# batra-mlp-lab/visdial

Hardware: AMD Instinct MI355X
Metric: QA-rounds/sec training mn-att-ques-im-hist+disc (batch 20x10x100) (higher is better)
Workload: dtype f32 operands and results; the option recurrence multiplies the EXACT 3-way bf16 split of both operands (9 bf16 MFMA products per fp32 product, f32 accumulate: fp32-grade, errors at the f32 MFMA's own level) -- its two step kernels and its weight-gradient contraction; f32 MFMA (v_mfma_f32_32x32x2_f32

## Files before the change

### visdial_amd/csrc/gemm_ops.hip

```cpp
#include "gemm_core.h"
#include "split_core.h"

using CfgBigDB = GemmCfg<4, 1, 4, 32>;
using CfgBig = GemmCfg<4, 1, 4, 16, 0, 3>;
using CfgSmall = GemmCfg<1, 4, 1, 32, 0, 3>;

static inline bool use_small(int M, int N) {
  return (long)vd_cdiv(M, CfgBig::BM) * vd_cdiv(N, CfgBig::BN) < 48;
}

static int check_align(const void* p, long ld, const char* what) {
  if (((uintptr_t)p & 15) != 0 || (ld & 3) != 0) {
    vd_set_error("%s: pointer must be 16-byte aligned and leading dimension a multiple of 4 (ld=%ld)", what, ld);
    return VD_ERR_ARG;
  }
  return VD_OK;
}

__global__ void colsum_kernel(const float* __restrict__ X, long ld, int M, int N, int rows_per_block,
                              float* __restrict__ out) {
  const int col = blockIdx.x * blockDim.x + threadIdx.x;
  if (col >= N) return;
  const int r0 = blockIdx.y * rows_per_block;
  const int r1 = min(M, r0 + rows_per_block);
// ... 349 lines not shown
  const int* tok_mask;
  static constexpr bool HAS_DEAD = true;
  __device__ __forceinline__ bool dead(int row_base, int ) const { return tok_mask[row_base] == 0; }
};
static_assert(CfgSmall::BM == VD_LSTM_FWD_TILE_SMALL && CfgBig::BM == VD_LSTM_FWD_TILE_BIG, "the projection's row tiles are the step kernels'");

int vd_gemm_nn_live_p(const float* A, int64_t lda, const float* B, int64_t ldb, const float* bias, float* C, int64_t ldc, int M, int N, int K,
                      const int32_t* tok_mask, int row_tile, hipStream_t s) {
  VD_CHECK_ARG(A && B && C && tok_mask && M >= 0 && N >= 0 && K >= 0 && (K % 4 == 0 || lda >= (K + 3) / 4 * 4) && N % 4 == 0 &&
                   (row_tile == CfgSmall::BM || row_tile == CfgBig::BM),
               "vd_gemm_nn (live rows): bad args M=%d N=%d K=%d row tile %d", M, N, K, row_tile);
  if (int rc = check_align(A, lda, "vd_gemm_nn (live rows) A")) return rc;
  if (int rc = check_align(B, ldb, "vd_gemm_nn (live rows) B")) return rc;
  SrcRow a{A, lda};
  SrcK b{B, ldb};
  if (row_tile == CfgSmall::BM) {
    EpiStoreLive<1> e{{C, ldc, bias, VD_ACT_NONE, 0}, tok_mask};
    return launch_gemm<CfgSmall>(M, N, K, 1, a, b, e, s);
  }
  EpiStoreLive<4> e{{C, ldc, bias, VD_ACT_NONE, 0}, tok_mask};
  return launch_gemm<CfgBig>(M, N, K, 1, a, b, e, s);
}

extern "C" {

int vd_gemm_tn_acc(const float* A, int64_t lda, const float* B, int64_t ldb, float* C, int64_t ldc, int M,
                   int N, int K, int flags, void* stream) {
  VD_CHECK_ARG(A && B && C && M >= 0 && N >= 0 && K >= 0 && (M % 4 == 0 || lda >= (M + 3) / 4 * 4) &&
                   (N % 4 == 0 || ldb >= (N + 3) / 4 * 4),
               "vd_gemm_tn_acc: bad args M=%d N=%d K=%d", M, N, K);
  if (int rc = check_align(A, lda, "vd_gemm_tn_acc A")) return rc;
  if (int rc = check_align(B, ldb, "vd_gemm_tn_acc B")) return rc;
  if (K == 0) return VD_OK;
  SrcK a{A, lda}, b{B, ldb};
  EpiAtomic<4> e{C, ldc};
  const long tiles = (long)vd_cdiv(M, CfgBig::BM) * vd_cdiv(N, CfgBig::BN);
  if ((flags & VD_FLAG_SPLIT9) && !(flags & VD_FLAG_BF16) && vd_tn_split_tiles(M, N) && K >= 8192 &&
      16L * lda * 4 < (1L << 31) && 16L * ldb * 4 < (1L << 31)) {
    const int K1 = K & ~15;
    if (int rc = launch_gemm_split_tn<9>(M, N, K1, A, lda, B, ldb, C, ldc, (hipStream_t)stream)) return rc;
    if (K1 == K) return VD_OK;
    SrcK a2{A + (long)K1 * lda, lda}, b2{B + (long)K1 * ldb, ldb};
    return launch_gemm<GemmCfg<4, 1, 4, 16, 0, 4, 41984>>(M, N, K - K1, 1, a2, b2, e, (hipStream_t)stream);
  }
  const bool kmaj = !(flags & VD_FLAG_BF16) && vd_tn_kmajor_fits(M, N, K);
  if (kmaj && K % 16 != 0) {
// ... 126 lines not shown
```

### visdial_amd/csrc/paths.h

```cpp
#pragma once
#include "common.h"

static inline int vd_precision_flags(int lstmBf16) {
  switch (lstmBf16) {
    case 0: return 0;
    case 1: return VD_FLAG_BF16;
    case 3: return VD_FLAG_SPLIT3;
    case 6: return VD_FLAG_SPLIT6;
    case 9: return VD_FLAG_SPLIT9;
    default: return -1;
  }
}
static inline int vd_split_nprod(int flags) {
  return (flags & VD_FLAG_SPLIT9) ? 9 : (flags & VD_FLAG_SPLIT6) ? 6 : (flags & VD_FLAG_SPLIT3) ? 3 : 0;
}

constexpr long VD_THROUGHPUT_ROWS = 2048;
constexpr int VD_LSTM_FWD_TILE_BIG = 128, VD_LSTM_FWD_TILE_SMALL = 32;
static inline int vd_lstm_fwd_row_tile(long N) { return N >= VD_THROUGHPUT_ROWS ? VD_LSTM_FWD_TILE_BIG : VD_LSTM_FWD_TILE_SMALL; }
static inline bool vd_lstm_glds_fwd_fits(long N, int H) { return N >= VD_THROUGHPUT_ROWS && H % 32 == 0 && N * H * 4 < (1L << 32); }
static inline bool vd_lstm_glds_bwd_fits(long N, int H) { return N >= VD_THROUGHPUT_ROWS && H % 32 == 0 && N * 4 * H * 4 < (1L << 32); }
static inline bool vd_lstm_bf16_fits(long N, int H) { return N >= VD_THROUGHPUT_ROWS && H % 32 == 0; }
static inline bool vd_lstm_c16_fits(long N, int H) { return N >= VD_THROUGHPUT_ROWS && H % 128 == 0; }

static inline bool vd_tn_kmajor_fits(long M, long N, long K) { return M % 128 == 0 && N % 128 == 0 && K >= 1024; }
constexpr int VD_SPLIT_TN_BM = 256, VD_SPLIT_TN_BN = 128;
static inline bool vd_tn_split_tiles(long M, long N) { return M % VD_SPLIT_TN_BM == 0 && N % VD_SPLIT_TN_BN == 0; }

static inline bool vd_wgrad_group_fits(bool sorted_rows, long M, long N, int flags) {
  return sorted_rows && M % 128 == 0 && N % 128 == 0 && !(flags & VD_FLAG_BF16);
}

static inline bool vd_img_split_ok(long rows, int H, int Kc) {
  return rows >= 128 && H % 16 == 0 && Kc % 16 == 0 && rows * (H > Kc ? H : Kc) * 4 < (1L << 32);
}

static inline bool vd_lhood_fused_fits(long rows, long ldh, long V, long ldw, int H) {
  return H >= 64 && H % 16 == 0 && V >= 128 && ldh % 4 == 0 && ldw % 4 == 0 && rows * ldh * 4 < (1L << 32) && V * ldw * 4 < (1L << 32);
}
static inline bool vd_lhood_prefix_fits(int T, long rows) { return T >= 1 && T < 256 && rows >= 1; }
```

### visdial_amd/csrc/rt_core.h

```cpp
#pragma once
#include <math.h>
#include <stdarg.h>
#include <stdlib.h>
#include <string.h>

#include <algorithm>
#include <map>
#include <memory>
#include <numeric>
#include <random>
#include <string>
#include <vector>

#include "../../include/visdial_hip.h"
#include "common.h"
#include "paths.h"
#include "rt_switches.h"
#include "wgrad_plan.h"

static_assert(VD_OK == 0 && VD_ERR_ARG == -1, "rt_switches.h returns the two as literals: it includes no common.h");

int vd_lstm2_forward_p(const vd_lstm2_fwd_t* st, int nstacks, int H, int flags, hipStream_t stream);
int vd_lstm2_backward_p(const vd_lstm2_bwd_t* st, int nstacks, int H, int flags, hipStream_t stream);

// ... 1 lines not shown
int vd_img_common_forward_p(const float* pre, const uint8_t* mask1, const float* xdrop, const float* Wc, const float* bc, const float* qc,
                            const uint8_t* mask2, float* iqc, int N, int R, int S2, int H, int Kc, float scale, int flags, hipStream_t stream);
int vd_img_tr_backward_p(const float* dz, const float* Wc, const float* p, const float* datt, const uint8_t* mask1, float* dpre, int N, int R,
                         int S2, int H, int Kc, float scale, int flags, hipStream_t stream);
int vd_img_common_wgrad_p(const float* dz, const float* pre, const uint8_t* mask1, const float* xdrop, float* dWc, int N, int R, int S2, int H,
                          int Kc, float scale, int flags, hipStream_t stream);

int vd_img_att_forward_p(const float* iqc, const float* wa, const float* ba, const float* pre, const uint8_t* mask1, const float* u0, float* p,
                         float* u1, int N, int R, int S2, int H, int Kc, float scale, const int32_t* cnt, hipStream_t stream);
int vd_img_att_backward_p(float* iqc_dz, const float* wa, const float* pre, const uint8_t* mask1, const uint8_t* mask2, const float* p,
                          const float* datt, float* dwa, float* dba, float* dqc, float* work, int N, int R, int S2, int H, int Kc, float scale,
                          const int32_t* cnt, hipStream_t stream);

int vd_mn_attention_round_p(const float* Q, int64_t q_ld, const float* Hm, float* P, float* hAtt, float* Qout, int B, int R, int r, int H,
                            hipStream_t stream);
int vd_hrea_attention_round_p(const float* sq, const float* sh, const float* Hm, float* P, float* att, int B, int R, int r, int H,
                              hipStream_t stream);
int vd_round_embed_p(const float* emb, const int32_t* tok, int T, int N, int R, int r, int32_t* tok_r, float* x, int E, hipStream_t stream);
int vd_rows_cat_p(float* dst, int64_t dst_ld, const float* const* src, const int64_t* ld, const int* cols, int nparts, int64_t rows,
                  hipStream_t stream);

int vd_gemm_nn_live_p(const float* A, int64_t lda, const float* B, int64_t ldb, const float* bias, float* C, int64_t ldc, int M, int N, int K,
                      const int32_t* tok_mask, int row_tile, hipStream_t stream);
int vd_lhood_order_p(const int32_t* tok_in, const int32_t* target, int T, int64_t rows, int C, int32_t* perm, int32_t* rep, int32_t* tok_in_s,
                     int32_t* target_s, int32_t* work, int32_t* info, hipStream_t stream);
int64_t vd_lhood_order_work_ints(int T, int64_t rows);
int vd_lhood_sum_p(const float* nll, const int32_t* act, int64_t n_act, int T, int64_t rows, int C, const int32_t* perm, float* out, int64_t ldo,
                   hipStream_t stream);

int vd_lhood_lse_p(const float* h, int64_t ldh, int64_t rows, const int32_t* act, int64_t n_act, const float* W, int64_t ldw, const float* bias,
                   int V, int H, float* lse, hipStream_t stream);
int vd_lhood_edge_sum_p(const float* h, int64_t ldh, const int32_t* node_row, const float* lse, const int32_t* enode, const int32_t* etgt, int T,
                        int64_t rows, int C, const float* W, int64_t ldw, const float* bias, int H, float* out, int64_t ldo, hipStream_t stream);

int vd_sample_draw_trunc_p(const float* logits, int64_t ld, int64_t rows, int V, int32_t* tok, const double* uniforms, double temperature,
                           int top_k, double top_p, int step, int beam_len, int end_token, int32_t* hist, double* loglik, int32_t* status,
                           hipStream_t stream);

int vd_beam_advance_p(const int32_t* top_idx, const float* top_val, int rounds, int k, int G, float lambda, int step, int beam_len,
                      int end_token, double* scores, const int32_t* hist_in, int32_t* hist_out, int32_t* src, int32_t* next_tok,
                      double* best_score, int32_t* best_len, int32_t* best_hist, const double* lp, hipStream_t stream);
int vd_beam_topk_ban_p(const float* logits, int64_t ld, int64_t rows, int V, const int32_t* tok, int k, const int32_t* hist, int beam_len,
                       int step, int min_len, int no_repeat, int end_token, int32_t* top_idx, float* top_val, hipStream_t stream);

int vd_beam_rollout_append_p(const int32_t* answers, int beam_len, int end_token, const int32_t* ques, int Tq, int dialogs, int R, int r,
                             int32_t* hist_tok, int32_t* hist_sorted, const int32_t* inv, int Th, hipStream_t stream, int concat_end = 0);
// ... 230 lines not shown
  return VD_OK;
}

template <class T>
int ws_get(vd_model* m, const std::string& key, size_t count, T** out) {
  void* p = nullptr;
  VD_TRY(dev_get(m->ws, key, count * sizeof(T), &p));
  *out = static_cast<T*>(p);
  return VD_OK;
}

inline void add_lstm(vd_model* m, const std::string& name, long D, long H) {
  m->spec.push_back(Tensor{name + ".W", 0, D + H, 4 * H, 1});
  m->spec.push_back(Tensor{name + ".b", 0, 1, 4 * H, 2});
}
inline void add_linear(vd_model* m, const std::string& name, long in, long out) {
  m->spec.push_back(Tensor{name + ".W", 0, out, in, 3});
  m->spec.push_back(Tensor{name + ".b", 0, 1, out, 4});
}
inline std::string hop_sfx(int i) { return i == 0 ? std::string() : std::to_string(i + 1); }

inline float* Wp(vd_model* m, const std::string& n) { return m->W + m->spec[m->index.at(n)].off; }
inline float* Gp(vd_model* m, const std::string& n) { return m->G + m->spec[m->index.at(n)].off; }

inline int fork_stream(vd_model* m, hipStream_t from, hipStream_t side) {
  if (side == from) return VD_OK;
  hipEvent_t e = m->ev_pool[m->ev_next++ % m->ev_pool.size()];
  VD_HIP(hipEventRecord(e, from));
  VD_HIP(hipStreamWaitEvent(side, e, 0));
  return VD_OK;
}
inline int join_stream(vd_model* m, hipStream_t side, hipStream_t to) { return fork_stream(m, side, to); }
inline hipStream_t side_stream(vd_model* m, hipStream_t cur) { return m->streams ? m->s_side : cur; }
inline int wg_fork(vd_model* m, hipStream_t cur, hipStream_t* out) {
  *out = cur;
  if (!m->wg_active || !m->s_wg) return VD_OK;
  VD_TRY(fork_stream(m, cur, m->s_wg));
  m->wg_used = true;
  *out = m->s_wg;
  return VD_OK;
}

constexpr int VD_WGRAD_CHUNKS = 768, VD_WGRAD_MIN_KSTEPS = 32;
inline void wgrad_begin(vd_model* m) {
  m->wgrad.clear();
  m->wgrad_open = true;
// ... 284 lines not shown
    if (T > 1 && grouped(h, H, gates + (long)N * 4 * H, dWh, 1)) {
    } else if (by_rows && !(T > 1 && dense_fits(H, (long)(T - 1) * N))) {
      if (rows->n_act1 > 0)
        VD_TRY(vd_gemm_tn_rows_acc(h, H, rows->prev1, gates, 4 * H, rows->act1, dWh, 4 * H, (int)H, (int)(4 * H), rows->n_act1, s));
    } else if (T > 1) {
      VD_TRY(vd_gemm_tn_acc(h, H, gates + (long)N * 4 * H, 4 * H, dWh, 4 * H, (int)H, (int)(4 * H), (T - 1) * N, wg_flags(H), s));
    }
    if (h0) VD_TRY(vd_gemm_tn_acc(h0, H, gates, 4 * H, dWh, 4 * H, (int)H, (int)(4 * H), N, 0, s));
    VD_TRY(vd_colsum_acc(gates, 4 * H, (int)TN, (int)(4 * H), Gp(m, name + ".b"), s));
    if (dxs) dxs->assign(parts.size(), nullptr);
    long roff = 0;
    for (size_t i = 0; i < parts.size(); ++i) {
      if (grouped(xs[i], parts[i], gates, dW + roff * 4 * H, 0)) {
      } else if (by_rows && !dense_fits(parts[i], TN)) {
        if (rows->n_act > 0)
          VD_TRY(vd_gemm_tn_rows_acc(xs[i], parts[i], rows->act, gates, 4 * H, rows->act, dW + roff * 4 * H, 4 * H, (int)parts[i],
                                     (int)(4 * H), rows->n_act, s));
      } else {
        VD_TRY(vd_gemm_tn_acc(xs[i], parts[i], gates, 4 * H, dW + roff * 4 * H, 4 * H, (int)parts[i], (int)(4 * H), (int)TN, wg_flags(parts[i]), s));
      }
      if (need_dx.empty() || need_dx[i]) {
        float* dx;
        VD_TRY(ws_get(m, name + ".dx" + std::to_string(i), (size_t)TN * parts[i], &dx));
        VD_TRY(vd_gemm_nt(gates, 4 * H, Wx(m) + roff * 4 * H, 4 * H, nullptr, dx, parts[i], (int)TN, (int)parts[i], (int)(4 * H),
                          VD_ACT_NONE, 0, s));
        if (dxs) (*dxs)[i] = dx;
      }
      roff += parts[i];
    }
    return VD_OK;
  }
  int backward(vd_model* m, hipStream_t s, const float* dh_seq, const float* dh_last, const std::vector<bool>& need_dx,
               std::vector<float*>* dxs) {
    if (gradPrevOutput) {
      if (!dh_last) dh_last = gradPrevOutput;
      else {
        float* t;
        VD_TRY(ws_get(m, name + ".dhl", (size_t)N * H, &t));
        VD_TRY(vd_axpby(dh_last, gradPrevOutput, t, (long)N * H, 1.f, 1.f, s));
        dh_last = t;
      }
    }
    const float* dc_last = userNextGradCell;
    gradPrevOutput = userNextGradCell = nullptr;
    float *dc, *dh0 = nullptr;
    VD_TRY(ws_get(m, name + ".dc", (size_t)N * H, &dc));
    if (h0) VD_TRY(ws_get(m, name + ".dh0", (size_t)N * H, &dh0));
    VD_TRY(vd_lstm_backward(Wh(m), gates, c, c0, dh_seq, dh_last, dc_last, dc, dh0, nullptr, nullptr, T, N, (int)H, 0, s));
// ... 28 lines not shown
```

### visdial_amd/csrc/rt_decoders.h

```cpp
#pragma once
#include "rt_encoders.h"

namespace vdrt {

int option_cache_resolve(vd_model* m, BatchSlot& sl, const int32_t* options, long NO, int To, hipStream_t s);

struct Decoder {
  virtual ~Decoder() {}
  virtual void declare(vd_model* m) = 0;
  virtual int forward_backward(vd_model* m, BatchSlot& b, bool only_forward) = 0;
  virtual int retrieve(vd_model* m, BatchSlot& b) = 0;
  virtual int retrieve_lhood(vd_model*, BatchSlot&) {
    vd_set_error("vd_model_retrieve_lhood: the live-row log-likelihood head scores candidates of decoder 'gen'; this model's decoder is 'disc'");
    return VD_ERR_ARG;
  }
  virtual int gen_begin(vd_model*, const int32_t*, int) { return no_gen(); }
  virtual int gen_step(vd_model*, const int32_t*, float*) { return no_gen(); }
  virtual int gen_select(vd_model*, const int32_t*, int) { return no_gen(); }
  virtual int gen_beam_search(vd_model*, int, int, int, int, int32_t*, double*) { return no_gen(); }
  virtual int gen_sample(vd_model*, int, int, int, double, const double*, int32_t*, double*) { return no_gen(); }
  static int no_gen() {
    vd_set_error("sampling / beam search only for the generative decoder (model.lua:436-438)");
    return VD_ERR_STATE;
  }
// ... 38 lines not shown
}
#define VD_PROBE_REC(i, stream) (void)hipEventRecord(probe_events()[i], stream)
#else
#define VD_PROBE_REC(i, stream)
#endif
struct Disc : Decoder {
  void declare(vd_model* m) override { add_lstm(m, "opt", m->p.embedSize, m->p.rnnHiddenSize); }
  struct OptStates {
    bool c16;
    float *table, *gates, *h, *c, *h_last;
    vd_bf16_bits *gates16, *h16;
    const float* optH;
  };
  int option_states(vd_model* m, const SeqTok& opt, OptStates* o) {
    const int NO = opt.N, To = opt.T;
    const long H = m->p.rnnHiddenSize, E = m->p.embedSize, V = m->p.vocabSize;
    hipStream_t s = m->s_main;
    VD_TRY(ws_get(m, "opt.table", (size_t)(V + 1) * 4 * H, &o->table));
    VD_TRY(ws_get(m, "opt.gates", (size_t)To * NO * 4 * H, &o->gates));
    VD_TRY(ws_get(m, "opt.h", (size_t)To * NO * H, &o->h));
    VD_TRY(ws_get(m, "opt.c", (size_t)To * NO * H, &o->c));
    float* Wopt = Wp(m, "opt.W");
    const int flags = m->flags;
    VD_TRY(vd_gemm_nn(Wp(m, "embed"), E, Wopt, 4 * H, Wp(m, "opt.b"), o->table, 4 * H, (int)V + 1, (int)(4 * H), (int)E, 0, s));
    o->c16 = (flags & VD_FLAG_BF16) && vd_lstm_c16_fits(NO, (int)H);
    o->gates16 = reinterpret_cast<vd_bf16_bits*>(o->gates);
    o->h16 = reinterpret_cast<vd_bf16_bits*>(o->h);
    o->h_last = nullptr;
    vd_bf16_bits* table16 = nullptr;
    if (o->c16) {
      float* t16;
      VD_TRY(ws_get(m, "opt.table16", (size_t)(V + 1) * 2 * H, &t16));
      VD_TRY(ws_get(m, "opt.h_last", (size_t)NO * H, &o->h_last));
      table16 = reinterpret_cast<vd_bf16_bits*>(t16);
      VD_TRY(vd_f32_to_bf16(o->table, table16, (V + 1) * 4 * H, s));
    }
    VD_HIP(hipEventRecord(m->ev_prof[0], s));
    {
      VdRange r("disc: option LSTM forward");
      if (o->c16) VD_TRY(vd_lstm_forward_c16(table16, 4 * H, opt.tok, Wopt + E * 4 * H, o->gates16, o->h16, o->h_last, o->c, To, NO, (int)H, s));
      else VD_TRY(vd_lstm_forward(o->table, 0, 4 * H, opt.tok, nullptr, Wopt + E * 4 * H, nullptr, nullptr, o->gates, o->h, o->c, To, NO, (int)H, flags, s));
    }
    VD_HIP(hipEventRecord(m->ev_prof[1], s));
    o->optH = o->c16 ? o->h_last : o->h + (long)(To - 1) * NO * H;
    return VD_OK;
  }
  int option_states_full(vd_model* m, BatchSlot& b, const OptStates& o, const float** optH) {
// ... 101 lines not shown
      VdRange r("disc: option LSTM backward");
      if (c16) VD_TRY(vd_lstm_backward_c16(Wopt + E * 4 * H, gates16, c, d_optH, dc, To, NO, (int)H, s));
      else VD_TRY(vd_lstm_backward(Wopt + E * 4 * H, gates, c, nullptr, nullptr, d_optH, nullptr, dc, nullptr, nullptr, nullptr, To, NO, (int)H, flags, s));
    }
    VD_HIP(hipEventRecord(m->ev_prof[3], s));
    VD_TRY(enc_bwd());
    VdRange rwg("disc: table gradient + dWh");
    VD_TRY(fork_stream(m, s, sd));
    if (!m->wgrad.empty()) {
      VD_TRY(wgrad_flush(m, b, sd));
      VD_HIP(hipEventRecord(m->ev_enc_grads, sd));
    }
    if (c16) VD_TRY(vd_segment_rowsum_acc_bf16(gates16, 4 * H, opt.tok, perm, (long)To * NO, (int)(4 * H), dtab, 4 * H, sd));
    else VD_TRY(vd_segment_rowsum_acc(gates, 4 * H, opt.tok, perm, (long)To * NO, (int)(4 * H), dtab, 4 * H, sd));
    VD_TRY(vd_colsum_acc(dtab, 4 * H, (int)V + 1, (int)(4 * H), Gp(m, "opt.b"), sd));
    VD_TRY(vd_gemm_tn_acc(Wp(m, "embed"), E, dtab, 4 * H, Gp(m, "opt.W"), 4 * H, (int)E, (int)(4 * H), (int)V + 1, 0, sd));
    VD_HIP(hipEventRecord(m->ev_prof[4], s));
    if (To > 1 && c16)
      VD_TRY(vd_gemm_tn_acc_bf16(h16, gates16 + (long)NO * 4 * H, Gp(m, "opt.W") + E * 4 * H, 4 * H, (int)H, (int)(4 * H), (To - 1) * NO, s));
    else if (To > 1)
      VD_TRY(vd_gemm_tn_acc(h, H, gates + (long)NO * 4 * H, 4 * H, Gp(m, "opt.W") + E * 4 * H, 4 * H, (int)H, (int)(4 * H), (To - 1) * NO,
                            flags & (VD_FLAG_BF16 | VD_FLAG_SPLIT9), s));
    VD_HIP(hipEventRecord(m->ev_prof[5], s));
    VD_TRY(vd_gemm_nt(dtab, 4 * H, Wopt, 4 * H, nullptr, Gp(m, "embed"), E, (int)V + 1, (int)E, (int)(4 * H), VD_ACT_NONE, 2, sd));
    VD_PROBE_REC(3, sd);
    VD_TRY(join_stream(m, sd, s));
    if (m->wg_used) VD_TRY(join_stream(m, m->s_wg, s));
    m->wg_active = m->wg_used = false;
    VD_PROBE_REC(4, s);
    return VD_OK;
  }
  int retrieve(vd_model* m, BatchSlot& b) override {
    if (m->sw.retrieve_rollout && m->use_hist) return retrieve_rollout(m, b);
    return forward_backward(m, b, true);
  }

  int retrieve_rollout(vd_model* m, BatchSlot& b) {
    VD_TRY(refuse_round_rollout_in_training(m, "vd_model_retrieve"));
    if (m->training) {
      vd_set_error("vd_model_retrieve: this model was created with VD_RETRIEVE_ROLLOUT = 1, and a rollout re-runs the encoder once per round: "
                   "under training-mode dropout the passes would not describe one model; call vd_model_set_training(0) first");
      return VD_ERR_STATE;
    }
    VD_CHECK_ARG(b.opt.present && !b.cached, "decoder 'disc' needs batch.options");
    const int N = b.q.N, O = m->p.numOptions, NOfull = N * O, NO = b.opt.N, R = m->p.maxQuesCount, B = N / R;
    const bool dedup = b.opt_uid != nullptr;
    VD_CHECK_ARG(dedup ? NO <= NOfull : NO == NOfull, "decoder 'disc': %d option rows for %d x %d candidates", NO, N, O);
// ... 691 lines not shown
```

### visdial_amd/csrc/rt_encoders.h

```cpp
#pragma once
#include "rt_core.h"

namespace vdrt {

struct Encoder {
  virtual ~Encoder() {}
  virtual void declare(vd_model* m) = 0;
  virtual int forward(vd_model* m, hipStream_t s, BatchSlot& b, float** out) = 0;
  virtual int backward(vd_model* m, hipStream_t s, BatchSlot& b, const float* grad_out) = 0;
  virtual int forward_round(vd_model* m, hipStream_t s, BatchSlot& b, int r, float** out) {
    vd_set_error("encoder '%s' has no history: a rollout never asks it for a round pass", m->enc_name.c_str());
    return VD_ERR_STATE;
  }
  float* out_ = nullptr;
  int round_ready(vd_model* m, const BatchSlot& b, bool state = true) const {
    const int N = b.q.N, R = m->p.maxQuesCount;
    VD_CHECK_ARG(out_ && state && N == N / R * R && b.h.N == N, "round pass without a full encoder pass on this batch");
    return VD_OK;
  }
  virtual std::vector<SeqLSTM>* rnnLayers() { return nullptr; }
  virtual int seqLen(const BatchSlot& b) const { return b.q.T; }
};

inline int tick_flags(const vd_model* m) { return m->flags & VD_FLAG_BF16; }
// ... 14 lines not shown
  return VD_OK;
}

struct WaveStack {
  SeqLSTM *l1 = nullptr, *l2 = nullptr;
  std::string tag;
  bool drop = false;
  uint8_t* mask = nullptr;

  int prepare(vd_model* m, hipStream_t s, const SeqTok& ss) {
    VD_CHECK_ARG(ss.sorted, "the '%s' stack (%s, %s) runs on length-sorted rows only", tag.c_str(), l1->name.c_str(), l2->name.c_str());
    const long E = l1->D, H = l1->H;
    const long TN = (long)ss.T * ss.N;
    mask = nullptr;
    if (drop) VD_TRY(drop_mask(m, tag + "_emb", (size_t)TN * E, 0.5f, s, &mask));
    float *x, *xs;
    VD_TRY(ws_get(m, tag + ".x", (size_t)TN * E, &x));
    VD_TRY(ws_get(m, tag + ".xs", (size_t)TN * E, &xs));
    VD_TRY(l1->alloc(m, ss.T, ss.N));
    VD_TRY(l2->alloc(m, ss.T, ss.N));
    l1->h0 = l1->c0 = l2->h0 = l2->c0 = nullptr;
    VD_TRY(vd_embed_gather(Wp(m, "embed"), ss.tok, mask, x, TN, (int)E, drop ? 2.0f : 1.0f, s));
    VD_TRY(vd_embed_gather(x, ss.fwd_idx, nullptr, xs, TN, (int)E, 1.0f, s));
    VD_TRY(vd_gemm_nn(xs, E, l1->Wx(m), 4 * H, Wp(m, l1->name + ".b"), l1->gates, 4 * H, (int)TN, (int)(4 * H), (int)E, 0, s));
    VdZeroSet z{{l1->gates, l1->h, l1->c, l2->h, l2->c, l2->gates}, {(int)(4 * H), (int)H, (int)H, (int)H, (int)H, (int)(4 * H)}, 6, 0};
    VD_TRY(vd_zero_inactive_multi(z, ss.nact_dev, ss.T, ss.N, s));
    l1->xs = {xs};
    l2->xs = {l1->h};
    l1->rows = l2->rows = &ss;
    return VD_OK;
  }
  static void fill_fwd(vd_model* m, const SeqLSTM& l1, const SeqLSTM& l2, int T, int N, const int32_t* tok_mask, const int32_t* nact,
                       float* const* gates, float* const* h, float* const* c, vd_lstm2_fwd_t* o) {
    o->T = T; o->N = N;
    o->tok_mask = tok_mask;
    o->Wh1 = l1.Wh(m); o->Wx2 = l2.Wx(m); o->b2 = Wp(m, l2.name + ".b"); o->Wh2 = l2.Wh(m);
    o->gates1 = gates[0]; o->h1 = h[0]; o->c1 = c[0]; o->gates2 = gates[1]; o->h2 = h[1]; o->c2 = c[1];
    o->nact = nact;
  }
  void fill_fwd(vd_model* m, const SeqTok& ss, vd_lstm2_fwd_t* o) const {
    float *gates[2] = {l1->gates, l2->gates}, *h[2] = {l1->h, l2->h}, *c[2] = {l1->c, l2->c};
    fill_fwd(m, *l1, *l2, ss.T, ss.N, ss.tok_sorted, ss.nact.data(), gates, h, c, o);
  }
  int fill_bwd(vd_model* m, const SeqTok& ss, const float* dlast, vd_lstm2_bwd_t* o) const {
    const long H = l1->H;
    float *dhseq, *dc1, *dc2;
    VD_TRY(ws_get(m, l1->name + ".dhseq", (size_t)ss.T * ss.N * H, &dhseq));
// ... 815 lines not shown
```

### visdial_amd/csrc/rt_switches.h

```cpp
#pragma once
#include <errno.h>
#include <float.h>
#include <stdint.h>
#include <stdlib.h>
#include <string.h>

#include <string>

void vd_set_error(const char* fmt, ...);

namespace vdrt {

static constexpr long VD_OPTION_CACHE_DEFAULT_ROWS = 262144;

struct Switches {
  long option_cache_rows = 0;
  bool lhood_tree = false;
  int sample_topk = 0;
  double sample_topp = 1.0;
  int beam_groups = 1;
  double beam_diversity = 0.5;
  int beam_min_len = 0, beam_no_repeat = 0;
  double beam_length_penalty = 0.0;
  bool beam_rollout = false, retrieve_rollout = false;
  bool rollout_round = false;
  int rollout_concat_end = 0;
  double label_smoothing = 0.0;
  double grad_clip_norm = 0.0;
  double weight_decay = 0.0;
  double dense_mix = 0.0;
};

inline bool switch_refused(const char* name, const char* e, const char* must) {
  vd_set_error("vd_model_create: %s = '%s' %s", name, e, must);
  return false;
}
inline bool read_int(const char* name, long lo, const char* must, int* out) {
  const char* e = getenv(name);
  if (!e) return true;
  char* end = nullptr;
  errno = 0;
  const long v = strtol(e, &end, 10);
  if (!(*e && end && !*end && errno == 0 && v >= lo && v <= INT32_MAX)) return switch_refused(name, e, must);
  *out = (int)v;
  return true;
}
inline bool read_real(const char* name, double lo, bool lo_open, double hi, const char* must, double* out) {
  const char* e = getenv(name);
  if (!e) return true;
  char* end = nullptr;
  const double v = strtod(e, &end);
  if (!(*e && end && !*end && (lo_open ? v > lo : v >= lo) && v <= hi)) return switch_refused(name, e, must);
  *out = v;
// ... 42 lines not shown
                  "among a round's groups is the host's", sw.beam_groups);
  if (disc && !read_choice("VD_RETRIEVE_ROLLOUT", "0", "1", flag, &sw.retrieve_rollout)) return -1;
  VD_SWITCH_NEEDS(!sw.retrieve_rollout || sw.option_cache_rows == 0,
                  "vd_model_create: VD_RETRIEVE_ROLLOUT = 1 with VD_OPTION_CACHE: a cached batch carries only the candidate rows the cache did "
                  "not hold, and the rollout reads a picked candidate's tokens from the batch; combining the two is left for a follow-up");
#undef VD_SWITCH_NEEDS
  bool round = false;
  if (!read_choice("VD_ROLLOUT_ENCODER", "full", "round", "must be 'full' or 'round' (unset = full)", &round)) return -1;
  sw.rollout_round = round && (sw.beam_rollout || sw.retrieve_rollout) && strstr(encoder, "hist");
  if (!read_int("VD_ROLLOUT_CONCAT_END", 0, "must be an integer >= 0: the <END> token id (0 = off)", &sw.rollout_concat_end)) return -1;
  if (!((sw.beam_rollout || sw.retrieve_rollout) && strstr(encoder, "hist"))) sw.rollout_concat_end = 0;
  if (sw.rollout_concat_end && strncmp(encoder, "lf-", 3))
    return vd_set_error("vd_model_create: VD_ROLLOUT_CONCAT_END = %d with encoder '%s': its history is one row per round (beam.hip R2 / E4), not "
                        "the running concatenation of the dialog; the concatenation rule (CH1-CH6) is for lf-ques-hist, lf-ques-im-hist and "
                        "lf-att-ques-im-hist", sw.rollout_concat_end, encoder), -1;
  const char* real0 = "must be a finite real >= 0 (0 = off)";
  if (!(read_real("VD_LABEL_SMOOTHING", 0.0, false, 1.0 - (double)FLT_EPSILON / 2, "must be a real in [0, 1) (0 = off)", &sw.label_smoothing) &&
        read_real("VD_GRAD_CLIP_NORM", 0.0, false, (double)FLT_MAX, real0, &sw.grad_clip_norm) &&
        read_real("VD_WEIGHT_DECAY", 0.0, false, (double)FLT_MAX, real0, &sw.weight_decay)))
    return -1;
  if (!read_real("VD_DENSE_MIX", 0.0, false, 1.0, "must be a finite real in [0, 1] (0 = rounds without an annotation do not train)",
                 &sw.dense_mix))
    return -1;
  *out = sw;
  return 0;
}

}
```

### visdial_amd/csrc/split_core.h

```cpp
#pragma once
#include "gemm_core.h"
#include "paths.h"

typedef __bf16 vd_bf16x8 __attribute__((ext_vector_type(8)));

__device__ __forceinline__ unsigned vd_cvt_pk_bf16(float a, float b) {
  unsigned r;
  asm("v_cvt_pk_bf16_f32 %0, %1, %2" : "=v"(r) : "v"(a), "v"(b));
  return r;
}
__device__ __forceinline__ float vd_bf16_lo_f32(unsigned p) {
  float r;
  asm("v_lshlrev_b32 %0, 16, %1" : "=v"(r) : "v"(p));
  return r;
}
__device__ __forceinline__ float vd_bf16_hi_f32(unsigned p) {
  float r;
  asm("v_and_b32 %0, 0xffff0000, %1" : "=v"(r) : "v"(p));
  return r;
}
__device__ __forceinline__ float vd_sub_f32(float a, float b) {
  float r;
  asm("v_sub_f32 %0, %1, %2" : "=v"(r) : "v"(a), "v"(b));
  return r;
// ... 12 lines not shown
  vd_split3_pair(u.z, u.w, h[1], m[1], l[1]);
  vd_split3_pair(w.x, w.y, h[2], m[2], l[2]);
  vd_split3_pair(w.z, w.w, h[3], m[3], l[3]);
  hi = __builtin_bit_cast(vd_bf16x8, (vd_u32x4){h[0], h[1], h[2], h[3]});
  mid = __builtin_bit_cast(vd_bf16x8, (vd_u32x4){m[0], m[1], m[2], m[3]});
  lo = __builtin_bit_cast(vd_bf16x8, (vd_u32x4){l[0], l[1], l[2], l[3]});
}

static __global__ void __launch_bounds__(256) f32_to_bf16x3_kernel(const float* __restrict__ src, vd_bf16_bits* __restrict__ dst, long n4, long plane) {
  const long i = (long)blockIdx.x * 256 + threadIdx.x;
  if (i >= n4) return;
  const float4 v = reinterpret_cast<const float4*>(src)[i];
  float4 r1, r2;
  typedef __bf16 bf4 __attribute__((ext_vector_type(4)));
  const bf4 h = {(__bf16)v.x, (__bf16)v.y, (__bf16)v.z, (__bf16)v.w};
  r1.x = v.x - (float)h[0]; r1.y = v.y - (float)h[1]; r1.z = v.z - (float)h[2]; r1.w = v.w - (float)h[3];
  const bf4 m = {(__bf16)r1.x, (__bf16)r1.y, (__bf16)r1.z, (__bf16)r1.w};
  r2.x = r1.x - (float)m[0]; r2.y = r1.y - (float)m[1]; r2.z = r1.z - (float)m[2]; r2.w = r1.w - (float)m[3];
  const bf4 l = {(__bf16)r2.x, (__bf16)r2.y, (__bf16)r2.z, (__bf16)r2.w};
  *reinterpret_cast<bf4*>(dst + i * 4) = h;
  *reinterpret_cast<bf4*>(dst + plane + i * 4) = m;
  *reinterpret_cast<bf4*>(dst + 2 * plane + i * 4) = l;
}
static int weights_to_bf16x3(const float* src, vd_bf16_bits* dst, long n, hipStream_t s) {
  hipLaunchKernelGGL(f32_to_bf16x3_kernel, dim3((unsigned)((n / 4 + 255) / 256)), dim3(256), 0, s, src, dst, n / 4, n);
  VD_LAUNCH_CHECK();
  return VD_OK;
}

struct SplitCfg {
    static constexpr int NT = 4, WM = 4, THREADS = 64 * WM;
  static constexpr int BM = 32 * WM, BN = 128, KS = 32;
  static constexpr int BTILE = BN * 64;
  static constexpr int STAGE = 3 * BTILE;
  static constexpr int LDS_BYTES = 2 * STAGE;
  static constexpr int SCR = LDS_BYTES / WM / 4;
  static_assert(SCR >= 32 * QUAD_LD, "quad_to_tile's 32 rows of QUAD_LD floats");
};

#ifndef VD_SPLIT_CG
#define VD_SPLIT_CG 2
#endif
static_assert(VD_SPLIT_CG >= 1 && VD_SPLIT_CG <= 8 && 8 % VD_SPLIT_CG == 0, "the XCD grid is VD_SPLIT_CG x (8 / VD_SPLIT_CG)");
__device__ __forceinline__ bool split_tile_of(int bid, int nwg, int tiles_m, int tiles_n, int& tile_m, int& tile_n) {
  constexpr int CG = VD_SPLIT_CG, RG = 8 / CG;
  if ((tiles_n % CG) == 0 && tiles_n >= 8) {
    const int xcd = bid & 7, li = bid >> 3, cpg = tiles_n / CG, rpg = (tiles_m + RG - 1) / RG;
    tile_n = (xcd % CG) * cpg + li % cpg;
    tile_m = (xcd / CG) * rpg + li / cpg;
    return tile_m < tiles_m && li / cpg < rpg;
  }
  const int wg = xcd_remap(bid, nwg);
  tile_n = wg % tiles_n;
  tile_m = wg / tiles_n;
  return true;
}
__device__ __forceinline__ int split_swz(int q) { return (0x78 >> (2 * (q & 3))) & 3; }
static int split_grid(int tiles_m, int tiles_n) {
  constexpr int CG = VD_SPLIT_CG, RG = 8 / CG;
  if ((tiles_n % CG) == 0 && tiles_n >= 8) return 8 * ((tiles_m + RG - 1) / RG) * (tiles_n / CG);
  return tiles_m * tiles_n;
}

template <int NPROD, class Epi>
__global__ void __launch_bounds__(SplitCfg::THREADS, 3)
gemm_split_kernel(int M, int N, int K, int tiles_n, const float* A, long lda, const vd_bf16_bits* B, long ldb, long bplane, Epi epi) {
  using Cfg = SplitCfg;
  constexpr int NT = Cfg::NT;
  extern __shared__ __attribute__((aligned(16))) float smem[];
  int tile_m, tile_n;
  if (!split_tile_of((int)blockIdx.x, (int)gridDim.x, (M + Cfg::BM - 1) / Cfg::BM, tiles_n, tile_m, tile_n)) return;
  const int row_base = tile_m * Cfg::BM, col_base = tile_n * Cfg::BN;
  constexpr int NIB = 24 / Cfg::WM;
  const int tid = (int)threadIdx.x, lane = tid & 63;
  const int wm = __builtin_amdgcn_readfirstlane(tid >> 6);
  const int nfull = K / 32, nm = nfull + ((K >> 4) & 1);
  const int wrow = row_base + wm * 32;
  const int g = lane >> 4, l15 = lane & 15;

  vd_f32x4 acc[2][2 * NT];
#pragma unroll
  for (int rt = 0; rt < 2; ++rt)
#pragma unroll
    for (int j = 0; j < 2 * NT; ++j)
#pragma unroll
      for (int r = 0; r < 4; ++r) acc[rt][j][r] = 0.f;

  typename EpiPreOf<Epi>::type pre;
  if constexpr (EpiPreOf<Epi>::value) epi.preload(pre, wrow, lane, M);

  unsigned aoff[2];
#pragma unroll
  for (int rt = 0; rt < 2; ++rt) aoff[rt] = (unsigned)(((long)min(wrow + rt * 16 + l15, M - 1) * lda + g * 8) * 4);
  float4 an[2][2];
  auto load_a = [&](int m) {
    const char* ak = reinterpret_cast<const char*>(A + (long)m * 32);
    const bool live = m < nfull || g < 2;
#pragma unroll
    for (int rt = 0; rt < 2; ++rt) {
      an[rt][0] = an[rt][1] = make_float4(0.f, 0.f, 0.f, 0.f);
      if (live) {
        an[rt][0] = *reinterpret_cast<const float4*>(ak + aoff[rt]);
        an[rt][1] = *reinterpret_cast<const float4*>(ak + aoff[rt] + 16);
      }
    }
  };
  const int csrc = (lane & 3) ^ split_swz(lane >> 4);
  unsigned voffb[NIB];
#pragma unroll
  for (int i = 0; i < NIB; ++i) {
    const int r = ((wm * NIB + i) & 7) * 16 + (lane >> 2);
    voffb[i] = (unsigned)(((long)min(col_base + r, N - 1) * ldb + csrc * 8) * 2);
  }
  const unsigned lds0 = (unsigned)(uintptr_t)smem;
  auto issue_b = [&](int m, int st) {
    const unsigned back = m < nfull ? 0u : (unsigned)(csrc >> 1) * 32u;
#pragma unroll
    for (int i = 0; i < NIB; ++i) {
      const int q = wm * NIB + i;
      glds16(voffb[i] - back, reinterpret_cast<const float*>(B + (long)(q >> 3) * bplane + (long)m * 32), lds0 + st * Cfg::STAGE + q * 1024);
    }
  };
  const int bfrag = l15 * 64 + ((g ^ split_swz(l15 >> 2)) * 16);

  auto load_a_full = [&](int m) {
    const char* ak = reinterpret_cast<const char*>(A + (long)m * 32);
#pragma unroll
    for (int rt = 0; rt < 2; ++rt) {
      an[rt][0] = *reinterpret_cast<const float4*>(ak + aoff[rt]);
      an[rt][1] = *reinterpret_cast<const float4*>(ak + aoff[rt] + 16);
    }
  };
  auto issue_b_full = [&](int m, int st) {
#pragma unroll
    for (int i = 0; i < NIB; ++i) {
      const int q = wm * NIB + i;
      glds16(voffb[i], reinterpret_cast<const float*>(B + (long)(q >> 3) * bplane + (long)m * 32), lds0 + st * Cfg::STAGE + q * 1024);
    }
  };
// ... 40 lines not shown
  if (nm > 0) {
    issue_b(0, 0);
    load_a(0);
    int m = 0;
    for (; m + 1 < nfull; ++m) step(m, m & 1, std::true_type{});
    if (m < nm) {
      step(m, m & 1, std::false_type{});
      if (++m < nm) step(m, m & 1, std::false_type{});
    }
  }
  float* scr = smem + wm * Cfg::SCR;
  f32x16 tile[NT];
#pragma unroll
  for (int j = 0; j < NT; ++j) tile[j] = quad_to_tile(acc[0][2 * j], acc[0][2 * j + 1], acc[1][2 * j], acc[1][2 * j + 1], scr, lane);
  if constexpr (EpiPreOf<Epi>::value) epi(tile, wrow, col_base, lane, M, N, scr, &pre);
  else epi(tile, wrow, col_base, lane, M, N, scr);
}

template <int NPROD, class Epi>
static int launch_gemm_split(int M, int N, int K, const float* A, long lda, const vd_bf16_bits* B, long ldb, long bplane, const Epi& e,
                             hipStream_t stream) {
  if (M <= 0 || N <= 0) return VD_OK;
  using Cfg = SplitCfg;
  VD_CHECK_ARG(K % 16 == 0 && lda % 4 == 0 && ldb % 8 == 0 && (long)M * lda * 4 < (1L << 32) && (long)N * ldb * 2 < (1L << 32),
               "launch_gemm_split: unsupported shape M=%d N=%d K=%d", M, N, K);
  const int tiles_m = vd_cdiv(M, Cfg::BM), tiles_n = vd_cdiv(N, Cfg::BN);
  auto kern = gemm_split_kernel<NPROD, Epi>;
  static bool attr_set = false;
  if (!attr_set) {
    VD_HIP(hipFuncSetAttribute(reinterpret_cast<const void*>(kern), hipFuncAttributeMaxDynamicSharedMemorySize, 160 * 1024));
    attr_set = true;
  }
  hipLaunchKernelGGL(kern, dim3(split_grid(tiles_m, tiles_n)), dim3(Cfg::THREADS), Cfg::LDS_BYTES, stream, M, N, K, tiles_n, A, lda, B, ldb, bplane, e);
  VD_LAUNCH_CHECK();
  return VD_OK;
}

template <class Epi>
static int launch_gemm_split(int nprod, int M, int N, int K, const float* A, long lda, const vd_bf16_bits* B, long ldb, long bplane,
                             const Epi& e, hipStream_t stream) {
  if (nprod == 9) return launch_gemm_split<9>(M, N, K, A, lda, B, ldb, bplane, e, stream);
  if (nprod == 6) return launch_gemm_split<6>(M, N, K, A, lda, B, ldb, bplane, e, stream);
  return launch_gemm_split<3>(M, N, K, A, lda, B, ldb, bplane, e, stream);
}

struct SplitTnCfg {
  static constexpr int BM = 256, BN = 128, THREADS = 256;
// ... 146 lines not shown
```

Before: 9432.

## Route dense embedding and input-projection GEMMs through 9-product bf16 split kernel

Adds split-plane conversion kernels and dense NN/NT wrappers so the embedding-table, LSTM input-projection and dx GEMMs use the exact 3-way bf16 split MFMA kernel instead of the f32 MFMA GEMM when SPLIT9 is set. An epilogue hook lets the split kernel skip tiles whose rows are all inactive in length-sorted sequences, optionally zeroing them. The split kernel is generalized to K multiples of 4. The cost is an extra per-call weight split pass into scratch and 9 MFMA products per output; the path is on by default via a new switch.

Result: no change. 9502, median of 6 (+0.7%).

```diff
diff --git a/visdial_amd/csrc/gemm_ops.hip b/visdial_amd/csrc/gemm_ops.hip
--- a/visdial_amd/csrc/gemm_ops.hip
+++ b/visdial_amd/csrc/gemm_ops.hip
@@ -395,6 +395,58 @@
   return launch_gemm<CfgBig>(M, N, K, 1, a, b, e, s);
 }
 
+struct EpiStoreRows : EpiStore<4> {
+  const int* nact;
+  int rows_per_step, zero_dead;
+  static constexpr bool SPLIT_LIVE = true;
+  __device__ __forceinline__ bool dead_tile(int row_base, int BM, int M) const {
+    if (!nact) return false;
+    const int r1 = min(row_base + BM, M);
+    for (int t = row_base / rows_per_step; t * rows_per_step < r1; ++t)
+      if (max(row_base - t * rows_per_step, 0) < nact[t]) return false;
+    return true;
+  }
+  __device__ __forceinline__ void leave(int row_base, int col_base, int tid, int BM, int BN, int M, int N) const {
+    if (!zero_dead || accumulate) return;
+    const int rows = min(BM, M - row_base), cols = min(BN, N - col_base);
+    for (int i = tid; i < rows * cols; i += SplitCfg::THREADS) C[(long)(row_base + i / cols) * ldc + col_base + i % cols] = 0.f;
+  }
+};
+
+static int dense_split_planes(hipStream_t stream, long N, int K, vd_bf16_bits** W3, long* K32) {
+  *K32 = (K + 31) / 32 * 32;
+  VdStreamScratch scr;
+  if (int rc = vd_stream_scratch(stream, (size_t)N * *K32 * 6, 0, &scr)) return rc;
+  *W3 = reinterpret_cast<vd_bf16_bits*>(scr.wht);
+  return VD_OK;
+}
+
+int vd_gemm_nn_split_p(const float* A, int64_t lda, const float* B, int64_t ldb, const float* bias, float* C, int64_t ldc, int M, int N, int K,
+                       const int32_t* nact, int rows_per_step, int zero_dead, int flags, hipStream_t stream) {
+  if (!(flags & VD_FLAG_SPLIT9) || !A || !B || !C || ((uintptr_t)A & 15) || !vd_dense_split_ok(M, N, K, lda) ||
+      (nact && (rows_per_step <= 0 || M % rows_per_step != 0)))
+    return vd_gemm_nn(A, lda, B, ldb, bias, C, ldc, M, N, K, 0, stream);
+  vd_bf16_bits* W3;
+  long K32;
+  if (int rc = dense_split_planes(stream, N, K, &W3, &K32)) return rc;
+  if (int rc = split_planes_cols(B, ldb, W3, K, N, stream)) return rc;
+  EpiStoreRows e{{C, ldc, bias, VD_ACT_NONE, 0}, nact, rows_per_step, zero_dead};
+  return launch_gemm_split<9>(M, N, K, A, lda, W3, K32, (long)N * K32, e, stream);
+}
+
+int vd_gemm_nt_split_p(const float* A, int64_t lda, const float* W, int64_t ldw, float* C, int64_t ldc, int M, int N, int K, int accumulate,
+                       const int32_t* nact, int rows_per_step, int zero_dead, int flags, hipStream_t stream) {
+  if (!(flags & VD_FLAG_SPLIT9) || !A || !W || !C || ((uintptr_t)A & 15) || ((uintptr_t)W & 15) || ldw % 4 != 0 || !vd_dense_split_ok(M, N, K, lda) ||
+      (nact && (rows_per_step <= 0 || M % rows_per_step != 0)))
+    return vd_gemm_nt(A, lda, W, ldw, nullptr, C, ldc, M, N, K, VD_ACT_NONE, accumulate, stream);
+  vd_bf16_bits* W3;
+  long K32;
+  if (int rc = dense_split_planes(stream, N, K, &W3, &K32)) return rc;
+  if (int rc = split_planes_rows(W, ldw, W3, N, K, stream)) return rc;
+  EpiStoreRows e{{C, ldc, nullptr, VD_ACT_NONE, accumulate}, nact, rows_per_step, zero_dead};
+  return launch_gemm_split<9>(M, N, K, A, lda, W3, K32, (long)N * K32, e, stream);
+}
+
 extern "C" {
 
 int vd_gemm_tn_acc(const float* A, int64_t lda, const float* B, int64_t ldb, float* C, int64_t ldc, int M,
diff --git a/visdial_amd/csrc/paths.h b/visdial_amd/csrc/paths.h
--- a/visdial_amd/csrc/paths.h
+++ b/visdial_amd/csrc/paths.h
@@ -35,6 +35,12 @@
   return rows >= 128 && H % 16 == 0 && Kc % 16 == 0 && rows * (H > Kc ? H : Kc) * 4 < (1L << 32);
 }
 
+static inline bool vd_dense_split_ok(long rows, long N, long K, long lda) {
+  const long K32 = (K + 31) / 32 * 32;
+  return rows >= VD_THROUGHPUT_ROWS && rows < (1L << 31) && N >= 1 && K >= 4 && K % 4 == 0 && lda % 4 == 0 && lda >= K && rows * lda * 4 < (1L << 32) &&
+         N * K32 * 2 < (1L << 32);
+}
+
 static inline bool vd_lhood_fused_fits(long rows, long ldh, long V, long ldw, int H) {
   return H >= 64 && H % 16 == 0 && V >= 128 && ldh % 4 == 0 && ldw % 4 == 0 && rows * ldh * 4 < (1L << 32) && V * ldw * 4 < (1L << 32);
 }
diff --git a/visdial_amd/csrc/rt_core.h b/visdial_amd/csrc/rt_core.h
--- a/visdial_amd/csrc/rt_core.h
+++ b/visdial_amd/csrc/rt_core.h
@@ -47,6 +47,10 @@
 
 int vd_gemm_nn_live_p(const float* A, int64_t lda, const float* B, int64_t ldb, const float* bias, float* C, int64_t ldc, int M, int N, int K,
                       const int32_t* tok_mask, int row_tile, hipStream_t stream);
+int vd_gemm_nn_split_p(const float* A, int64_t lda, const float* B, int64_t ldb, const float* bias, float* C, int64_t ldc, int M, int N, int K,
+                       const int32_t* nact, int rows_per_step, int zero_dead, int flags, hipStream_t stream);
+int vd_gemm_nt_split_p(const float* A, int64_t lda, const float* W, int64_t ldw, float* C, int64_t ldc, int M, int N, int K, int accumulate,
+                       const int32_t* nact, int rows_per_step, int zero_dead, int flags, hipStream_t stream);
 int vd_lhood_order_p(const int32_t* tok_in, const int32_t* target, int T, int64_t rows, int C, int32_t* perm, int32_t* rep, int32_t* tok_in_s,
                      int32_t* target_s, int32_t* work, int32_t* info, hipStream_t stream);
 int64_t vd_lhood_order_work_ints(int T, int64_t rows);
@@ -323,6 +327,7 @@
 
 inline float* Wp(vd_model* m, const std::string& n) { return m->W + m->spec[m->index.at(n)].off; }
 inline float* Gp(vd_model* m, const std::string& n) { return m->G + m->spec[m->index.at(n)].off; }
+inline int dense_flags(const vd_model* m) { return m->sw.dense_split ? m->flags : 0; }
 
 inline int fork_stream(vd_model* m, hipStream_t from, hipStream_t side) {
   if (side == from) return VD_OK;
@@ -653,8 +658,12 @@
       if (need_dx.empty() || need_dx[i]) {
         float* dx;
         VD_TRY(ws_get(m, name + ".dx" + std::to_string(i), (size_t)TN * parts[i], &dx));
-        VD_TRY(vd_gemm_nt(gates, 4 * H, Wx(m) + roff * 4 * H, 4 * H, nullptr, dx, parts[i], (int)TN, (int)parts[i], (int)(4 * H),
-                          VD_ACT_NONE, 0, s));
+        if (rows && rows->sorted && rows->nact_dev)
+          VD_TRY(vd_gemm_nt_split_p(gates, 4 * H, Wx(m) + roff * 4 * H, 4 * H, dx, parts[i], (int)TN, (int)parts[i], (int)(4 * H), 0, rows->nact_dev,
+                                    N, 1, dense_flags(m), s));
+        else
+          VD_TRY(vd_gemm_nt(gates, 4 * H, Wx(m) + roff * 4 * H, 4 * H, nullptr, dx, parts[i], (int)TN, (int)parts[i], (int)(4 * H),
+                            VD_ACT_NONE, 0, s));
         if (dxs) (*dxs)[i] = dx;
       }
       roff += parts[i];
diff --git a/visdial_amd/csrc/rt_decoders.h b/visdial_amd/csrc/rt_decoders.h
--- a/visdial_amd/csrc/rt_decoders.h
+++ b/visdial_amd/csrc/rt_decoders.h
@@ -84,7 +84,8 @@
     VD_TRY(ws_get(m, "opt.c", (size_t)To * NO * H, &o->c));
     float* Wopt = Wp(m, "opt.W");
     const int flags = m->flags;
-    VD_TRY(vd_gemm_nn(Wp(m, "embed"), E, Wopt, 4 * H, Wp(m, "opt.b"), o->table, 4 * H, (int)V + 1, (int)(4 * H), (int)E, 0, s));
+    VD_TRY(vd_gemm_nn_split_p(Wp(m, "embed"), E, Wopt, 4 * H, Wp(m, "opt.b"), o->table, 4 * H, (int)V + 1, (int)(4 * H), (int)E, nullptr, 0, 0,
+                              dense_flags(m), s));
     o->c16 = (flags & VD_FLAG_BF16) && vd_lstm_c16_fits(NO, (int)H);
     o->gates16 = reinterpret_cast<vd_bf16_bits*>(o->gates);
     o->h16 = reinterpret_cast<vd_bf16_bits*>(o->h);
@@ -232,7 +233,7 @@
       VD_TRY(vd_gemm_tn_acc(h, H, gates + (long)NO * 4 * H, 4 * H, Gp(m, "opt.W") + E * 4 * H, 4 * H, (int)H, (int)(4 * H), (To - 1) * NO,
                             flags & (VD_FLAG_BF16 | VD_FLAG_SPLIT9), s));
     VD_HIP(hipEventRecord(m->ev_prof[5], s));
-    VD_TRY(vd_gemm_nt(dtab, 4 * H, Wopt, 4 * H, nullptr, Gp(m, "embed"), E, (int)V + 1, (int)E, (int)(4 * H), VD_ACT_NONE, 2, sd));
+    VD_TRY(vd_gemm_nt_split_p(dtab, 4 * H, Wopt, 4 * H, Gp(m, "embed"), E, (int)V + 1, (int)E, (int)(4 * H), 2, nullptr, 0, 0, dense_flags(m), sd));
     VD_PROBE_REC(3, sd);
     VD_TRY(join_stream(m, sd, s));
     if (m->wg_used) VD_TRY(join_stream(m, m->s_wg, s));
diff --git a/visdial_amd/csrc/rt_encoders.h b/visdial_amd/csrc/rt_encoders.h
--- a/visdial_amd/csrc/rt_encoders.h
+++ b/visdial_amd/csrc/rt_encoders.h
@@ -60,7 +60,8 @@
     l1->h0 = l1->c0 = l2->h0 = l2->c0 = nullptr;
     VD_TRY(vd_embed_gather(Wp(m, "embed"), ss.tok, mask, x, TN, (int)E, drop ? 2.0f : 1.0f, s));
     VD_TRY(vd_embed_gather(x, ss.fwd_idx, nullptr, xs, TN, (int)E, 1.0f, s));
-    VD_TRY(vd_gemm_nn(xs, E, l1->Wx(m), 4 * H, Wp(m, l1->name + ".b"), l1->gates, 4 * H, (int)TN, (int)(4 * H), (int)E, 0, s));
+    VD_TRY(vd_gemm_nn_split_p(xs, E, l1->Wx(m), 4 * H, Wp(m, l1->name + ".b"), l1->gates, 4 * H, (int)TN, (int)(4 * H), (int)E, ss.nact_dev, ss.N, 0,
+                              dense_flags(m), s));
     VdZeroSet z{{l1->gates, l1->h, l1->c, l2->h, l2->c, l2->gates}, {(int)(4 * H), (int)H, (int)H, (int)H, (int)H, (int)(4 * H)}, 6, 0};
     VD_TRY(vd_zero_inactive_multi(z, ss.nact_dev, ss.T, ss.N, s));
     l1->xs = {xs};
diff --git a/visdial_amd/csrc/rt_switches.h b/visdial_amd/csrc/rt_switches.h
--- a/visdial_amd/csrc/rt_switches.h
+++ b/visdial_amd/csrc/rt_switches.h
@@ -29,6 +29,7 @@
   double grad_clip_norm = 0.0;
   double weight_decay = 0.0;
   double dense_mix = 0.0;
+  bool dense_split = true;
 };
 
 inline bool switch_refused(const char* name, const char* e, const char* must) {
@@ -117,6 +118,7 @@
   if (!read_real("VD_DENSE_MIX", 0.0, false, 1.0, "must be a finite real in [0, 1] (0 = rounds without an annotation do not train)",
                  &sw.dense_mix))
     return -1;
+  if (!read_choice("VD_DENSE_SPLIT", "0", "1", "must be 1 or 0 (unset = 1)", &sw.dense_split)) return -1;
   *out = sw;
   return 0;
 }
diff --git a/visdial_amd/csrc/split_core.h b/visdial_amd/csrc/split_core.h
--- a/visdial_amd/csrc/split_core.h
+++ b/visdial_amd/csrc/split_core.h
@@ -58,6 +58,59 @@
   *reinterpret_cast<bf4*>(dst + plane + i * 4) = m;
   *reinterpret_cast<bf4*>(dst + 2 * plane + i * 4) = l;
 }
+typedef __bf16 vd_bf16x4 __attribute__((ext_vector_type(4)));
+__device__ __forceinline__ void split3_store4(const float4& v, vd_bf16_bits* dst, long plane) {
+  float4 r1, r2;
+  const vd_bf16x4 h = {(__bf16)v.x, (__bf16)v.y, (__bf16)v.z, (__bf16)v.w};
+  r1.x = v.x - (float)h[0]; r1.y = v.y - (float)h[1]; r1.z = v.z - (float)h[2]; r1.w = v.w - (float)h[3];
+  const vd_bf16x4 m = {(__bf16)r1.x, (__bf16)r1.y, (__bf16)r1.z, (__bf16)r1.w};
+  r2.x = r1.x - (float)m[0]; r2.y = r1.y - (float)m[1]; r2.z = r1.z - (float)m[2]; r2.w = r1.w - (float)m[3];
+  const vd_bf16x4 l = {(__bf16)r2.x, (__bf16)r2.y, (__bf16)r2.z, (__bf16)r2.w};
+  *reinterpret_cast<vd_bf16x4*>(dst) = h;
+  *reinterpret_cast<vd_bf16x4*>(dst + plane) = m;
+  *reinterpret_cast<vd_bf16x4*>(dst + 2 * plane) = l;
+}
+static __global__ void __launch_bounds__(256) split_planes_rows_kernel(const float* __restrict__ src, long ld, vd_bf16_bits* __restrict__ dst, long rows,
+                                                                       int K, int K32, long plane) {
+  const long i = (long)blockIdx.x * 256 + threadIdx.x;
+  const int n4 = K32 / 4;
+  if (i >= rows * n4) return;
+  const long r = i / n4;
+  const int k = (int)(i - r * n4) * 4;
+  const float4 v = k < K ? *reinterpret_cast<const float4*>(src + r * ld + k) : make_float4(0.f, 0.f, 0.f, 0.f);
+  split3_store4(v, dst + r * K32 + k, plane);
+}
+static __global__ void __launch_bounds__(256) split_planes_cols_kernel(const float* __restrict__ src, long ld, vd_bf16_bits* __restrict__ dst, int K, int N,
+                                                                       int K32, long plane) {
+  __shared__ float tile[32][33];
+  const int tx = threadIdx.x & 31, ty = threadIdx.x >> 5;
+  const int k0 = blockIdx.y * 32, n0 = blockIdx.x * 32;
+#pragma unroll
+  for (int i = 0; i < 4; ++i) {
+    const int k = k0 + ty + i * 8, n = n0 + tx;
+    tile[ty + i * 8][tx] = (k < K && n < N) ? src[(long)k * ld + n] : 0.f;
+  }
+  __syncthreads();
+  const int nl = threadIdx.x >> 3, kk = (threadIdx.x & 7) * 4;
+  if (n0 + nl >= N) return;
+  const float4 v = make_float4(tile[kk][nl], tile[kk + 1][nl], tile[kk + 2][nl], tile[kk + 3][nl]);
+  split3_store4(v, dst + (long)(n0 + nl) * K32 + k0 + kk, plane);
+}
+static int split_planes_rows(const float* src, long ld, vd_bf16_bits* dst, long rows, int K, hipStream_t s) {
+  const int K32 = (K + 31) / 32 * 32;
+  const long n = rows * (K32 / 4);
+  if (n == 0) return VD_OK;
+  hipLaunchKernelGGL(split_planes_rows_kernel, dim3((unsigned)((n + 255) / 256)), dim3(256), 0, s, src, ld, dst, rows, K, K32, rows * K32);
+  VD_LAUNCH_CHECK();
+  return VD_OK;
+}
+static int split_planes_cols(const float* src, long ld, vd_bf16_bits* dst, int K, int N, hipStream_t s) {
+  const int K32 = (K + 31) / 32 * 32;
+  if (N == 0 || K32 == 0) return VD_OK;
+  hipLaunchKernelGGL(split_planes_cols_kernel, dim3((unsigned)((N + 31) / 32), (unsigned)(K32 / 32)), dim3(256), 0, s, src, ld, dst, K, N, K32, (long)N * K32);
+  VD_LAUNCH_CHECK();
+  return VD_OK;
+}
 static int weights_to_bf16x3(const float* src, vd_bf16_bits* dst, long n, hipStream_t s) {
   hipLaunchKernelGGL(f32_to_bf16x3_kernel, dim3((unsigned)((n / 4 + 255) / 256)), dim3(256), 0, s, src, dst, n / 4, n);
   VD_LAUNCH_CHECK();
@@ -98,6 +151,15 @@
   return tiles_m * tiles_n;
 }
 
+template <class Epi, class = void>
+struct EpiSplitLiveOf {
+  static constexpr bool value = false;
+};
+template <class Epi>
+struct EpiSplitLiveOf<Epi, std::void_t<decltype(Epi::SPLIT_LIVE)>> {
+  static constexpr bool value = Epi::SPLIT_LIVE;
+};
+
 template <int NPROD, class Epi>
 __global__ void __launch_bounds__(SplitCfg::THREADS, 3)
 gemm_split_kernel(int M, int N, int K, int tiles_n, const float* A, long lda, const vd_bf16_bits* B, long ldb, long bplane, Epi epi) {
@@ -107,10 +169,16 @@
   int tile_m, tile_n;
   if (!split_tile_of((int)blockIdx.x, (int)gridDim.x, (M + Cfg::BM - 1) / Cfg::BM, tiles_n, tile_m, tile_n)) return;
   const int row_base = tile_m * Cfg::BM, col_base = tile_n * Cfg::BN;
+  if constexpr (EpiSplitLiveOf<Epi>::value) {
+    if (epi.dead_tile(row_base, Cfg::BM, M)) {
+      epi.leave(row_base, col_base, (int)threadIdx.x, Cfg::BM, Cfg::BN, M, N);
+      return;
+    }
+  }
   constexpr int NIB = 24 / Cfg::WM;
   const int tid = (int)threadIdx.x, lane = tid & 63;
   const int wm = __builtin_amdgcn_readfirstlane(tid >> 6);
-  const int nfull = K / 32, nm = nfull + ((K >> 4) & 1);
+  const int nfull = K / 32, nm = (K + 31) / 32;
   const int wrow = row_base + wm * 32;
   const int g = lane >> 4, l15 = lane & 15;
 
@@ -131,14 +199,12 @@
   float4 an[2][2];
   auto load_a = [&](int m) {
     const char* ak = reinterpret_cast<const char*>(A + (long)m * 32);
-    const bool live = m < nfull || g < 2;
+    const int k0 = m * 32 + g * 8;
 #pragma unroll
     for (int rt = 0; rt < 2; ++rt) {
       an[rt][0] = an[rt][1] = make_float4(0.f, 0.f, 0.f, 0.f);
-      if (live) {
-        an[rt][0] = *reinterpret_cast<const float4*>(ak + aoff[rt]);
-        an[rt][1] = *reinterpret_cast<const float4*>(ak + aoff[rt] + 16);
-      }
+      if (k0 + 4 <= K) an[rt][0] = *reinterpret_cast<const float4*>(ak + aoff[rt]);
+      if (k0 + 8 <= K) an[rt][1] = *reinterpret_cast<const float4*>(ak + aoff[rt] + 16);
     }
   };
   const int csrc = (lane & 3) ^ split_swz(lane >> 4);
@@ -150,7 +216,7 @@
   }
   const unsigned lds0 = (unsigned)(uintptr_t)smem;
   auto issue_b = [&](int m, int st) {
-    const unsigned back = m < nfull ? 0u : (unsigned)(csrc >> 1) * 32u;
+    const unsigned back = (m < nfull || (K & 15)) ? 0u : (unsigned)(csrc >> 1) * 32u;
 #pragma unroll
     for (int i = 0; i < NIB; ++i) {
       const int q = wm * NIB + i;
@@ -237,7 +303,7 @@
                              hipStream_t stream) {
   if (M <= 0 || N <= 0) return VD_OK;
   using Cfg = SplitCfg;
-  VD_CHECK_ARG(K % 16 == 0 && lda % 4 == 0 && ldb % 8 == 0 && (long)M * lda * 4 < (1L << 32) && (long)N * ldb * 2 < (1L << 32),
+  VD_CHECK_ARG(K % 4 == 0 && (K % 16 == 0 || ldb >= (K + 31) / 32 * 32) && lda % 4 == 0 && ldb % 8 == 0 && (long)M * lda * 4 < (1L << 32) && (long)N * ldb * 2 < (1L << 32),
                "launch_gemm_split: unsupported shape M=%d N=%d K=%d", M, N, K);
   const int tiles_m = vd_cdiv(M, Cfg::BM), tiles_n = vd_cdiv(N, Cfg::BN);
   auto kern = gemm_split_kernel<NPROD, Epi>;
```
